# mkofinas/aether

Hardware: AMD Instinct MI355X
Metric: edge-messages/sec (forward, electrostatic N=20 batch=128 per GPU) (higher is better)
Workload: dtype f32; 1 GPU; electrostatic-2d-N20-B128; num_dims=2, nodes_per_graph=20, graphs_per_gpu=128, edges_per_gpu=48640, hidden=64, launch=hipgraph (10 steps per replay), parallelism=graphs sharded over 1 rank(s), no forward collective

## Files before the change

### aether_amd/_lib.py

```python
from __future__ import annotations

import ctypes as C
import os

HERE = os.path.dirname(os.path.abspath(__file__))
LIB_PATH = os.path.join(HERE, "libaether_hip.so")

PARAM_FIELDS = [
    ("field_w0", "field_net.net.0.weight"), ("field_b0", "field_net.net.0.bias"),
    ("field_w2", "field_net.net.2.weight"), ("field_b2", "field_net.net.2.bias"),
    ("field_w4", "field_net.net.4.weight"), ("field_b4", "field_net.net.4.bias"),
    ("field_emb", "field_net.class_embedding.weight"),
    ("l1_msg_w0", "gnn.layer_1.message_fn.0.weight"), ("l1_msg_b0", "gnn.layer_1.message_fn.0.bias"),
    ("l1_msg_w2", "gnn.layer_1.message_fn.2.weight"), ("l1_msg_b2", "gnn.layer_1.message_fn.2.bias"),
    ("l1_res_w", "gnn.layer_1.res.weight"), ("l1_res_b", "gnn.layer_1.res.bias"),
    ("l1_upd_w0", "gnn.layer_1.update_fn.0.weight"), ("l1_upd_b0", "gnn.layer_1.update_fn.0.bias"),
    ("l1_upd_w2", "gnn.layer_1.update_fn.2.weight"), ("l1_upd_b2", "gnn.layer_1.update_fn.2.bias"),
    ("ln_msg_w0", "gnn.layer_{}.message_fn.0.weight"), ("ln_msg_b0", "gnn.layer_{}.message_fn.0.bias"),
    ("ln_msg_w2", "gnn.layer_{}.message_fn.2.weight"), ("ln_msg_b2", "gnn.layer_{}.message_fn.2.bias"),
    ("ln_upd_w0", "gnn.layer_{}.update_fn.0.weight"), ("ln_upd_b0", "gnn.layer_{}.update_fn.0.bias"),
    ("ln_upd_w2", "gnn.layer_{}.update_fn.2.weight"), ("ln_upd_b2", "gnn.layer_{}.update_fn.2.bias"),
    ("out_w0", "gnn.out_mlp.0.weight"), ("out_b0", "gnn.out_mlp.0.bias"),
    ("out_w3", "gnn.out_mlp.3.weight"), ("out_b3", "gnn.out_mlp.3.bias"),
    ("out_w6", "gnn.out_mlp.6.weight"), ("out_b6", "gnn.out_mlp.6.bias"),
# ... 203 lines not shown
                                   [C.c_int, C.c_int, C.c_int, C.c_int] + [C.c_void_p] * 4 + [C.c_size_t, C.c_void_p]),
    "aether_sim_charged": (C.c_int, [C.c_void_p, C.c_void_p, C.c_void_p, C.c_void_p, C.c_int64, C.c_int, C.c_int, C.c_int,
                                     C.c_double, C.c_double, C.c_double, C.c_int, C.c_void_p, C.c_double, C.c_void_p,
                                     C.c_void_p, C.c_void_p]),
    "aether_rollout_dynamic_field": (C.c_int, [C.c_void_p, C.c_void_p, C.c_int, C.c_int64, C.c_int64, C.c_int] +
                                     [C.c_void_p] * 6 + [C.c_size_t, C.c_void_p, C.c_void_p, C.c_int, C.c_float, C.c_int,
                                                         C.c_void_p]),
    "aether_s2s_encoder_features": (C.c_int, [C.c_void_p, C.c_int, C.c_int, C.c_int, C.c_int, C.c_int64, C.c_int64] +
                                    [C.c_void_p] * 7 + [C.c_size_t, C.c_void_p, C.c_void_p]),
    "aether_s2s_lstm_step": (C.c_int, [C.c_void_p] * 4 + [C.c_int, C.c_int, C.c_int64] + [C.c_void_p] * 7),
    "aether_s2s_mlp_head": (C.c_int, [C.c_void_p, C.c_void_p, C.c_int, C.c_int, C.c_int, C.c_int, C.c_int64,
                                      C.c_void_p, C.c_void_p, C.c_void_p, C.c_void_p]),
    "aether_s2s_gumbel_hard": (C.c_int, [C.c_void_p, C.c_void_p, C.c_float, C.c_int, C.c_int64, C.c_void_p,
                                         C.c_void_p]),
    "aether_dynamic_field": (C.c_int, [C.c_void_p, C.c_int, C.c_int64, C.c_int, C.c_void_p, C.c_void_p, C.c_void_p,
                                       C.c_void_p, C.c_void_p]),
    "aether_forward_field": (C.c_int, [C.POINTER(AetherParams), C.c_int, C.c_int64, C.c_int64, C.c_void_p, C.c_void_p,
                                       C.c_void_p, C.c_void_p, C.c_void_p, C.c_void_p, C.POINTER(AetherGraphInfo),
                                       C.c_void_p, C.c_size_t, C.c_void_p, C.c_int, C.c_void_p]),
    "aether_debug_fetch": (C.c_int64, [C.c_char_p, C.c_int, C.c_int64, C.c_int64, C.c_void_p,
                                       C.c_void_p, C.c_void_p]),
    "aether_debug_split": (C.c_int, [C.c_void_p, C.c_int] + [C.c_void_p] * 5),
    "aether_debug_fused_packed_edge": (C.c_int, [C.c_int, C.c_int]),
    "aether_workspace_bytes_h": (C.c_size_t, [C.c_int64, C.c_int64, C.c_int, C.c_int, C.c_int]),
    "aether_dropout_mask_offset_h": (C.c_size_t, [C.c_int64, C.c_int64, C.c_int, C.c_int]),
    "aether_forward_h": (C.c_int, [C.POINTER(AetherParams), C.c_int, C.c_int, C.c_int64, C.c_int64, C.c_void_p, C.c_void_p,
                                   C.c_void_p, C.c_void_p, C.c_void_p, C.c_void_p, C.POINTER(AetherGraphInfo),
                                   C.c_void_p, C.c_size_t, C.c_void_p, C.c_int, C.c_void_p]),
    "aether_backward_h": (C.c_int, [C.POINTER(AetherParams), C.POINTER(AetherParams), C.c_int, C.c_int, C.c_int64,
                                    C.c_int64, C.c_void_p, C.c_void_p, C.c_void_p, C.c_void_p,
                                    C.POINTER(AetherGraphInfo), C.c_void_p, C.c_size_t, C.c_void_p, C.c_void_p,
                                    C.c_void_p]),
    "aether_backward_inputs_h": (C.c_int, [C.POINTER(AetherParams), C.c_int, C.c_int, C.c_int64, C.c_int64, C.c_void_p,
                                           C.c_void_p, C.c_void_p, C.c_void_p, C.POINTER(AetherGraphInfo), C.c_void_p,
                                           C.c_size_t, C.c_void_p, C.c_void_p, C.c_void_p, C.c_void_p, C.c_void_p,
                                           C.c_void_p, C.c_void_p]),
    "aether_rollout_h": (C.c_int, [C.POINTER(AetherParams), C.c_int, C.c_int, C.c_int64, C.c_int64, C.c_void_p, C.c_void_p,
                                   C.c_void_p, C.c_void_p, C.POINTER(AetherGraphInfo), C.c_void_p, C.c_size_t,
                                   C.c_void_p, C.c_int, C.c_float, C.c_int, C.c_void_p]),
    "aether_rollout_dynamic_field_h": (C.c_int, [C.c_void_p, C.c_void_p, C.c_int, C.c_int, C.c_int64, C.c_int64, C.c_int] +
                                       [C.c_void_p] * 6 + [C.c_size_t, C.c_void_p, C.c_void_p, C.c_int, C.c_float, C.c_int,
                                                           C.c_void_p]),
    "aether_debug_fetch_h": (C.c_int64, [C.c_char_p, C.c_int, C.c_int, C.c_int64, C.c_int64, C.c_void_p, C.c_void_p,
                                         C.c_void_p]),
    "aether_rollout_train_workspace_bytes": (C.c_size_t, [C.c_int64, C.c_int64, C.c_int, C.c_int, C.c_int]),
    "aether_rollout_train_forward": (C.c_int, [C.POINTER(AetherParams), C.c_int, C.c_int, C.c_int64, C.c_int64, C.c_void_p,
# ... 91 lines not shown
```

### aether_amd/csrc/aether_hip.hip

```cpp

#include <hip/hip_runtime.h>
#include <hipcub/hipcub.hpp>

#include <cstdint>
#include <cstdio>
#include <cstring>

#include "common.h"
#include "streamed.h"
#include "fused.h"
#include "backward.h"
#include "fused_bwd.h"
#include "edge_acc.h"
#include "input_grad.h"
#include "rollout_bwd.h"
#include "wide.h"
#include "seq2seq.h"
#include "s2s_filter.h"
#include "s2s_step.h"
#include "s2s_markov.h"
#include "s2s_charges.h"
#include "s2s_locs.h"
#include "s2s_dnri.h"
#include "dynfield.h"
// ... 1518 lines not shown
    if (name[0] == 'x' && name[1] >= '0' && name[1] <= '4' && !name[2])
        return copy2d((const float*)(ws + W.x[name[1] - '0']), n_nodes, H, 0, H);
    if (name[0] == 'e' && name[1] >= '1' && name[1] <= '4' && !name[2])
        return copy2d((const float*)(ws + W.e[name[1] - '1']), n_edges, H, 0, H);
    if (!strcmp(name, "efeat"))
        return copy2d((const float*)(ws + W.feat), n_edges, FPAD, 0, FPAD);
    return fail(AETHER_EINVAL, "debug_fetch: unknown name");
}

int aether_debug_split(const float* x, int n_tiles, uint16_t* hi, uint16_t* lo, int* on, float* scale, float* y) {
    if (!x || !hi || !lo || !on || !scale || !y) return fail(AETHER_EINVAL, "debug_split: null pointer");
    if (n_tiles < 0) return fail(AETHER_EINVAL, "debug_split: n_tiles");
    if (n_tiles == 0) return AETHER_OK;
    k_debug_split<<<dim3(1), dim3(64 * DEBUG_SPLIT_WAVES), 0, nullptr>>>(x, n_tiles, hi, lo, on, scale, y);
    HIP_OK(hipGetLastError());
    return AETHER_OK;
}

int aether_debug_fused_packed_edge(int wave, int lane) {
    if (wave < 0 || wave >= FUSED_PACK_WAVES || lane < 0 || lane >= FUSED_PACK_LANES) return -1;
    return fused_packed_edge(wave, lane);
}

#include "host_wide.inc"
#include "host_rollout_train.inc"

}
```

### aether_amd/csrc/common.h

```cpp
#pragma once
#include <hip/hip_runtime.h>
#include <cstdint>
#include <type_traits>
#include "../../include/aether_hip.h"

namespace {

typedef float f32x4 __attribute__((ext_vector_type(4)));
typedef float f32x2 __attribute__((ext_vector_type(2)));

constexpr int H = AETHER_HIDDEN;
constexpr int LDW = H + 8;
constexpr int FPAD = 32;
constexpr int LDF = FPAD + 8;
constexpr int LDST = H + 4;
constexpr float PI_F = 3.14159274101257324f;
constexpr float TWO_PI_F = 6.28318548202514648f;
constexpr float EPS_F = 1e-7f;

__device__ __forceinline__ void lds_barrier() { asm volatile("s_waitcnt lgkmcnt(0)\n\ts_barrier" ::: "memory"); }

__device__ __forceinline__ f32x4 mfma16(float a, float b, f32x4 c) {
    return __builtin_amdgcn_mfma_f32_16x16x4f32(a, b, c, 0, 0, 0);
}
// ... 502 lines not shown
    float c = cosf(theta), s = sinf(theta);
    if constexpr (D == 2) {
        R[0][0] = c; R[0][1] = -s; R[1][0] = s; R[1][1] = c;
    } else {
        float rho = sqrtf(v[0] * v[0] + v[1] * v[1] + v[2] * v[2]);
        float cz = v[2] / (rho + EPS_F);
        cz = fminf(fmaxf(cz, -1.0f), 1.0f);
        float phi = acosf(cz);
        float cp = cosf(phi), sp = sinf(phi);
        R[0][0] = cp * c; R[0][1] = -s;  R[0][2] = sp * c;
        R[1][0] = cp * s; R[1][1] = c;   R[1][2] = sp * s;
        R[2][0] = -sp;    R[2][1] = 0.f; R[2][2] = cp;
    }
#pragma unroll
    for (int a = 0; a < D; ++a) {
        float sv = 0.f, sf = 0.f;
#pragma unroll
        for (int b = 0; b < D; ++b) { sv += R[b][a] * v[b]; sf += R[b][a] * f[b]; }
        cv[a] = sv; cf[a] = sf;
    }
}

template <int D>
__device__ __forceinline__ void edge_features(const float* __restrict__ nj,
                                              const float* __restrict__ nir,
                                              const float* __restrict__ ea, float* __restrict__ o) {
    using NI = NodeInfo<D>;
    constexpr int O = D * (D - 1) / 2;
    float rel[D], rrel[D], rv[D], rf[D];
#pragma unroll
    for (int d = 0; d < D; ++d) rel[d] = nj[NI::P + d] - nir[NI::P + d];
#pragma unroll
    for (int a = 0; a < D; ++a) {
        float s0 = 0.f, s1 = 0.f, s2 = 0.f;
#pragma unroll
        for (int b = 0; b < D; ++b) {
            float rba = nir[NI::R + b * D + a];
            s0 += rba * rel[b];
            s1 += rba * nj[NI::V + b];
            s2 += rba * nj[NI::F + b];
        }
        rrel[a] = s0; rv[a] = s1; rf[a] = s2;
    }
    auto M = [&](int a, int c) {
        float s = 0.f;
#pragma unroll
// ... 42 lines not shown
```

### aether_amd/csrc/fused.h

```cpp
#pragma once
#include "common.h"
#include "fused_layout.h"
#include "fused_graph.h"
#include "fused_handoff.h"

namespace {

struct FusedDebug {
    float* nodeinfo; float* x[5]; float* e[4];
    float* n[4]; float* ps[3]; float* pr[3]; float* feat;
    int* flags;
    int* errword;
    const float* wimg;
    float* stamps;
    StepExtras step;
};
constexpr int FUSED_STAMPS = 512;

#ifdef AETHER_FUSED_STAMPS
#define FUSED_STAMP(id)                                                                          \
    do {                                                                                         \
        if (tid == 0 && blockIdx.x < 4096)                                                       \
            dbg.stamps[blockIdx.x * FUSED_STAMPS + (id)] = (float)(wall_clock64() - t_entry) * 0.01f; \
    } while (0)
#define FUSED_WSTAMP(layer_, r_, k_)                                                              \
    do {                                                                                         \
        if ((layer_) == 2 && lane == 0 && blockIdx.x < 4096 && wave < 16)                        \
            dbg.stamps[blockIdx.x * FUSED_STAMPS + 64 + wave * 24 + (r_) * 8 + (k_)] =            \
                (float)(__builtin_amdgcn_s_memtime() - c_entry);                                 \
    } while (0)
#define FUSED_WSTAMP_ROWS(layer_, r_)                                                             \
    do {                                                                                         \
        if ((layer_) == 2 && lane == 0 && blockIdx.x < 4096 && wave < 16)                        \
            dbg.stamps[blockIdx.x * FUSED_STAMPS + 352 + wave * 4 + (r_)] =                       \
                (float)(__builtin_amdgcn_s_memtime() - c_entry);                                 \
    } while (0)
#define FUSED_PSTAMP(k_, dep_)                                                                    \
    do {                                                                                         \
        asm volatile("v_mov_b32 %0, %0" : "+v"(dep_));                                           \
        if (wave == 0 && lane == 0 && blockIdx.x < 4096)                                         \
            dbg.stamps[blockIdx.x * FUSED_STAMPS + 400 + (k_)] =                                  \
                (float)(__builtin_amdgcn_s_memtime() - c_entry);                                 \
    } while (0)
#else
#define FUSED_STAMP(id)
#define FUSED_WSTAMP(layer_, r_, k_)
#define FUSED_WSTAMP_ROWS(layer_, r_)
#define FUSED_PSTAMP(k_, dep_)
#endif

template <int D, int NW, int ROUNDS, bool KEEP, bool GRAN = false>
__global__ void __launch_bounds__(NW * 64)
k_fused(AetherParams P, const float* __restrict__ x, const float* __restrict__ vel,
        const float* __restrict__ charges, const float* __restrict__ edge_attr_orig,
        const int32_t* __restrict__ perm, const int32_t* __restrict__ send_s,
        const int32_t* __restrict__ recv_s, const int32_t* __restrict__ rowptr,
        const FusedWG* __restrict__ wgdesc, const uint32_t* __restrict__ trec, const int4* __restrict__ ledge,
        const int32_t* __restrict__ nrange, FusedDebug dbg, float* __restrict__ out) {
    constexpr bool keep = KEEP;
    using NI = NodeInfo<D>;
    using L = FusedLds<NW, ROUNDS>;
    constexpr int THREADS = NW * 64;
    constexpr int FIN = 2 * D + 16;
    static_assert(NW == 8 || NW == 12, "waves 0-7 run the node phase; NW == 12 adds four waves that run step 3 (DESIGN.md 4.1)");
    static_assert(NW == 8 || (ROUNDS == 1 && !KEEP), "the 12-wave kernel owns one tile per wave and saves nothing for the backward");
    static_assert(!GRAN || NW == 12, "granules are the 12-wave kernel's hand-off");
    constexpr bool LATE = NW == 12 || ROUNDS == 2;
    constexpr bool EARLY = NW == 12;
    extern __shared__ __attribute__((aligned(16))) float smem[];
    float* wA = smem + L::WA;
    float* wB = smem + L::WB;
// ... 28 lines not shown
        const int total = nw_frag + FUSED_CBLK / 256;
        const int wv = __builtin_amdgcn_readfirstlane(wave);
        __builtin_assume(wv >= 0 && wv < NW);
        const int g_img = fused_wimg_offset(layer_, 0), g_cb = fused_cblk_offset(layer_);
        const int l_cb = L::CBLK + (layer_ & 1) * FUSED_CBLK;
        constexpr int MAXF = (32 + FUSED_CBLK / 256 + NW - 1) / NW;
#pragma unroll
        for (int j = 0; j < MAXF; ++j) {
            const int f = wv + NW * j;
            if (f < total) {
                const int img = f < na_frag ? f * 256 : FUSED_WIMG + (f - na_frag) * 256;
                const int soff = f < nw_frag ? g_img + img : g_cb + (f - nw_frag) * 256;
                const int doff = f < nw_frag ? L::WA + img : l_cb + (f - nw_frag) * 256;
                __builtin_amdgcn_global_load_lds(dbg.wimg + soff + lane * 4, (__attribute__((address_space(3))) void*)(smem + doff), 16, 0, 0);
            }
        }
    };
    dma_images(1);
    FUSED_STAMP(1);

    constexpr int FR = ROUNDS < 2 ? ROUNDS : 2;
    constexpr bool PACKED = NW == 12;
    constexpr bool FIMG = NW == 12;
    const int f_local = PACKED ? fused_packed_edge(wave, lane) : 16 * (NW * (lane >> 4) + wave) + (lane & 15);
    const bool f_have = (PACKED ? wave < FUSED_PACK_WAVES && lane < FUSED_PACK_LANES : lane < 16 * FR) && f_local < m;
    int4 f_e = make_int4(0, 0, 0, 0);
    f32x2 f_ea = {0.0f, 0.0f};
    int4 t_e[ROUNDS];
    unsigned seg_ends[ROUNDS];
    unsigned seg_rows[ROUNDS][4];
    {
        const int wv = __builtin_amdgcn_readfirstlane(wave);
#pragma unroll
        for (int r = 0; r < ROUNDS; ++r) {
            const int stile = NW * r + wv;
            const uint32_t* rec = trec + (size_t)(wg.tile0 + (stile < n_tiles ? stile : 0)) * FUSED_TREC;
            seg_ends[r] = stile < n_tiles ? __builtin_amdgcn_readfirstlane(rec[0]) : 0u;
#pragma unroll
            for (int w = 0; w < 4; ++w) seg_rows[r][w] = __builtin_amdgcn_readfirstlane(rec[2 + w]);
        }
    }
    const int aslot = (tid >> 4) & (FUSED_MAX_NODES - 1), ac4 = (tid & 15) * 4;
    int4 nr_rec;
    const int4* own_desc = reinterpret_cast<const int4*>(wgdesc + blockIdx.x);
    const int4* le_base = m > 0 ? ledge + eb : own_desc;
    const int4* nr_base = n > 0 ? reinterpret_cast<const int4*>(nrange) + nb : own_desc;
// ... 36 lines not shown
            int64_t g;
            float pz[D], vz[D], ef[D];
            float ch;
            float zc[6][3], a1[2][6];
            f32x4 w2f[2][2], w4f[2], acc1[2], acc2[2];
            f32x4 acc3 = f32x4{0.f, 0.f, 0.f, 0.f};
            float ar[4][2];
            f32x4 acc0[4];
            f32x4 fimg[FIMG ? FUSED_FIMG_CHUNKS : 1];
            if constexpr (FIMG) {
                const auto fimg_rsrc = __builtin_amdgcn_make_buffer_rsrc(const_cast<float*>(dbg.wimg) + fused_fimg_offset(), 0, FUSED_FIMG * 4, 0x00020000);
                p_ext = dbg.step.ext_field ? dbg.step.ext_field : x;
                asm volatile("" :: "s"(fimg_rsrc), "s"(p_ext), "s"(x), "s"(vel), "s"(charges), "s"(le_base), "s"(nr_base),
                             "s"(ea_base), "s"(qattr));
                node = 16 * wave + i;
                live = node < nv;
                g = vb + (live ? node : 0);
                FUSED_PSTAMP(0, f_e.x);
#pragma unroll
                for (int d = 0; d < D; ++d) { pz[d] = x[g * D + d]; vz[d] = vel[g * D + d]; ef[d] = p_ext[g * D + d]; }
                ch = charges[g];
#pragma unroll
                for (int c = 0; c < FUSED_FIMG_CHUNKS; ++c)
                    fimg[c] = __builtin_bit_cast(f32x4, __builtin_amdgcn_raw_buffer_load_b128(fimg_rsrc, lane * 16, c * 1024, 0));
            } else {
                const float* p_emb = P.field_emb; const float* p_w0 = P.field_w0; const float* p_b0 = P.field_b0;
                const float* p_w2 = P.field_w2; const float* p_b2 = P.field_b2; const float* p_w4 = P.field_w4;
                const float* p_b4 = P.field_b4; const float* p_rb = P.l1_res_b; const float* p_rw = P.l1_res_w;
                p_ext = dbg.step.ext_field ? dbg.step.ext_field : x;
                asm volatile("" :: "s"(p_emb), "s"(p_w0), "s"(p_b0), "s"(p_w2), "s"(p_b2), "s"(p_w4), "s"(p_b4), "s"(p_rb),
                             "s"(p_rw), "s"(p_ext), "s"(x), "s"(vel), "s"(charges), "s"(le_base), "s"(nr_base), "s"(ea_base),
                             "s"(qattr));
                node = 16 * wave + i;
                live = node < nv;
                g = vb + (live ? node : 0);
                FUSED_PSTAMP(0, f_e.x);
#pragma unroll
                for (int d = 0; d < D; ++d) { pz[d] = x[g * D + d]; vz[d] = vel[g * D + d]; ef[d] = p_ext[g * D + d]; }
                ch = charges[g];
#pragma unroll
                for (int s4 = 0; s4 < 6; ++s4) {
                    const int k = 4 * s4 + q;
                    const int ke = (k >= 2 * D && k < FIN) ? k - 2 * D : 0, kw = k < FIN ? k : 0;
#pragma unroll
                    for (int c = 0; c < 3; ++c)
                        zc[s4][c] = (4 * s4 + 3 >= 2 * D && 4 * s4 < FIN) ? p_emb[c * 16 + ke] : 0.0f;
#pragma unroll
// ... 13 lines not shown
#pragma unroll
                for (int mb = 0; mb < 4; ++mb) {
                    acc0[mb] = ld4(p_rb + 16 * mb + 4 * q);
#pragma unroll
                    for (int s4 = 0; s4 < 2; ++s4)
                        ar[mb][s4] = 4 * s4 < 2 * D ? p_rw[(16 * mb + i) * 3 * D + D + (4 * s4 + q < 2 * D ? 4 * s4 + q : 0)] : 0.0f;
                }
            }
            index_stage_a();
            __builtin_amdgcn_sched_barrier(0);
            __builtin_amdgcn_s_waitcnt(0x0F70);
            __builtin_amdgcn_sched_barrier(0);
            FUSED_PSTAMP(1, f_e.x);
            auto landed = [](auto v) { asm volatile("" :: "v"(v)); };
            auto landed4 = [](const int4& v) { asm volatile("" :: "v"(v.x), "v"(v.y), "v"(v.z), "v"(v.w)); };
            landed4(f_e); landed4(nr_rec);
#pragma unroll
            for (int r = 0; r < ROUNDS; ++r) landed4(t_e[r]);
#pragma unroll
            for (int d = 0; d < D; ++d) { landed(pz[d]); landed(vz[d]); landed(ef[d]); }
            landed(ch);
            if constexpr (FIMG) {
#pragma unroll
                for (int c = 0; c < FUSED_FIMG_CHUNKS; ++c) landed(fimg[c]);
                auto slot = [&](int s) { return fimg[s >> 2][s & 3]; };
#pragma unroll
                for (int mb = 0; mb < 2; ++mb) {
                    acc1[mb] = fimg[FI_ACC1 / 4 + mb]; acc2[mb] = fimg[FI_ACC2 / 4 + mb];
#pragma unroll
                    for (int a = 0; a < 2; ++a) w2f[mb][a] = fimg[FI_W2F / 4 + 2 * mb + a];
#pragma unroll
                    for (int s4 = 0; s4 < 6; ++s4) a1[mb][s4] = slot(FI_A1 + 6 * mb + s4);
                }
#pragma unroll
                for (int a = 0; a < 2; ++a) w4f[a] = fimg[FI_W4F / 4 + a];
                acc3 = fimg[FI_ACC3 / 4];
#pragma unroll
                for (int s4 = 0; s4 < 6; ++s4)
#pragma unroll
                    for (int c = 0; c < 3; ++c) zc[s4][c] = slot(FI_ZC + 3 * s4 + c);
#pragma unroll
                for (int mb = 0; mb < 4; ++mb) {
                    acc0[mb] = fimg[FI_ACC0 / 4 + mb];
#pragma unroll
                    for (int s4 = 0; s4 < 2; ++s4) ar[mb][s4] = slot(FI_AR + 2 * mb + s4);
                }
            } else {
#pragma unroll
                for (int s4 = 0; s4 < 6; ++s4) {
#pragma unroll
                    for (int c = 0; c < 3; ++c)
                        if (4 * s4 + 3 >= 2 * D && 4 * s4 < FIN) landed(zc[s4][c]);
#pragma unroll
                    for (int mb = 0; mb < 2; ++mb)
                        if (4 * s4 < FIN) landed(a1[mb][s4]);
                }
#pragma unroll
                for (int mb = 0; mb < 2; ++mb) { landed(acc1[mb]); landed(acc2[mb]); landed(w2f[mb][0]); landed(w2f[mb][1]); }
                landed(w4f[0]); landed(w4f[1]);
#pragma unroll
                for (int r = 0; r < D; ++r) landed(acc3[r]);
#pragma unroll
                for (int mb = 0; mb < 4; ++mb) {
                    landed(acc0[mb]);
#pragma unroll
                    for (int s4 = 0; s4 < 2; ++s4)
                        if (4 * s4 < 2 * D) landed(ar[mb][s4]);
                }
#pragma unroll
// ... 23 lines not shown
#pragma unroll
                for (int d = 0; d < D; ++d) { zk = k == d ? pz[d] : zk; zk = k == D + d ? vz[d] : zk; }
#pragma unroll
                for (int mb = 0; mb < 2; ++mb) acc1[mb] = mfma16(a1[mb][s4], zk, acc1[mb]);
            }
            f32x4 hh[2];
#pragma unroll
            for (int mb = 0; mb < 2; ++mb) hh[mb] = silu4(acc1[mb]);
            asm volatile("" : "+v"(f_e.y), "+v"(f_e.z), "+v"(f_e.w) : "v"(hh[0][0]));
            f_ea = index_stage_b();
#pragma unroll
            for (int a = 0; a < 2; ++a)
#pragma unroll
                for (int b = 0; b < 4; ++b)
#pragma unroll
                    for (int mb = 0; mb < 2; ++mb) acc2[mb] = mfma16(w2f[mb][a][b], hh[a][b], acc2[mb]);
#pragma unroll
            for (int mb = 0; mb < 2; ++mb) hh[mb] = silu4(acc2[mb]);
#pragma unroll
            for (int a = 0; a < 2; ++a)
#pragma unroll
                for (int b = 0; b < 4; ++b) acc3 = mfma16(w4f[a][b], hh[a][b], acc3);
            FUSED_PSTAMP(2, acc3[0]);
            if (q == 0 && live) {
                float f[D], R[D][D], cv[D], cf[D];
#pragma unroll
                for (int d = 0; d < D; ++d)
                    f[d] = dbg.step.ext_field ? ef[d] : acc3[d];
                node_frame<D>(vz, f, R, cv, cf);
                float* ni = ninfo + node * 24;
#pragma unroll
                for (int d = 0; d < D; ++d) {
                    ni[NI::P + d] = pz[d]; ni[NI::V + d] = vz[d]; ni[NI::F + d] = f[d];
                    ni[NI::CV + d] = cv[d]; ni[NI::CF + d] = cf[d];
#pragma unroll
                    for (int e = 0; e < D; ++e) ni[NI::R + d * D + e] = R[d][e];
                }
                if (keep && node >= off && node < off + n) {
                    float* gni = dbg.nodeinfo + (int64_t)(vb + node) * NI::STRIDE;
#pragma unroll
                    for (int t = 0; t < NI::STRIDE; ++t) gni[t] = t < NI::CF + D ? ni[t] : 0.0f;
                }
            }
            __builtin_amdgcn_wave_barrier();
            FUSED_PSTAMP(3, acc3[0]);
#pragma unroll
            for (int s4 = 0; s4 < 2; ++s4) {
                const int k = 4 * s4 + q;
                const float rk = (live && k < 2 * D) ? ninfo[node * 24 + NI::CV + k] : 0.0f;
#pragma unroll
                for (int mb = 0; mb < 4; ++mb) acc0[mb] = mfma16(ar[mb][s4], rk, acc0[mb]);
            }
            const int own = node - off;
            if (own >= 0 && own < n) {
#pragma unroll
                for (int mb = 0; mb < 4; ++mb) {
                    st4(xbuf + own * LDW + 16 * mb + 4 * q, acc0[mb]);
                    if (keep) st4(dbg.x[0] + (int64_t)(nb + own) * H + 16 * mb + 4 * q, acc0[mb]);
                }
            }
            FUSED_PSTAMP(4, acc0[3][0]);
        } else {
            index_stage_a();
            index_select();
            f_ea = index_stage_b();
            for (int idx = tid - 64 * vtiles; idx < (FUSED_MAX_NODES - n) * (H / 4); idx += THREADS - 64 * vtiles)
                st4(xbuf + (n + (idx >> 4)) * LDW + (idx & 15) * 4, f32x4{0.f, 0.f, 0.f, 0.f});
        }
        asm volatile("s_waitcnt vmcnt(0)" ::: "memory");
        lds_barrier();
    }
    FUSED_STAMP(2);

    int sl[ROUNDS], rl[ROUNDS];
    f32x4 e[ROUNDS][4];
    int ke[KEEP ? ROUNDS : 1];
    {
        float* scratch = smem + L::FEAT + wave * (L::FEAT_ROWS * LDF);
#pragma unroll
        for (int r0 = 0; r0 < ROUNDS; r0 += 2) {
            constexpr int PASS = 2;
            const int nr_pass = ROUNDS - r0 < PASS ? ROUNDS - r0 : PASS;
            if (PACKED ? wave < FUSED_PACK_WAVES && lane < FUSED_PACK_LANES : lane < 16 * nr_pass) {
                const int r = r0 + (lane >> 4), ii = lane & 15;
                const int local = PACKED ? f_local : 16 * (NW * r + wave) + ii;
                float o[FPAD];
                if (local < m) {
                    const int4 le = r0 == 0 ? f_e : ledge[eb + local];
                    const int k = le.x, ks = le.y, kr = le.z;
                    const float* nj = ninfo + (ks - vb) * 24;
                    const float* nr = ninfo + (kr - vb) * 24;
                    float njl[NI::STRIDE], nrl[NI::STRIDE];
#pragma unroll
                    for (int t = 0; t < NI::STRIDE; ++t) { njl[t] = nj[t]; nrl[t] = nr[t]; }
                    float eal[2];
                    if (dbg.step.qattr) {
                        float d2 = 0.0f;
#pragma unroll
                        for (int d = 0; d < D; ++d) {
                            const float df = njl[NI::P + d] - nrl[NI::P + d];
                            d2 += df * df;
                        }
                        eal[0] = r0 == 0 ? f_ea[0] * f_ea[1] : dbg.step.qattr[ks] * dbg.step.qattr[kr];
                        eal[1] = sqrtf(d2);
                    } else if (r0 == 0) {
                        eal[0] = f_ea[0]; eal[1] = f_ea[1];
                    } else {
                        const float* ea = edge_attr_orig + 2 * (int64_t)le.w;
                        eal[0] = ea[0]; eal[1] = ea[1];
                    }
                    edge_features<D>(njl, nrl, eal, o);
                } else {
#pragma unroll
                    for (int t = 0; t < FPAD; ++t) o[t] = 0.0f;
                }
#pragma unroll
                for (int t = 0; t < FPAD; t += 4)
// ... 601 lines not shown
```

### aether_amd/csrc/fused_layout.h

```cpp
#pragma once
#include "common.h"

namespace {

constexpr int FUSED_MAX_NODES = 32;
constexpr int FUSED_MAX_EDGES = 384;
constexpr int FUSED_MAX_TILES = FUSED_MAX_EDGES / 16;
constexpr int LDU = 2 * H + 8;
constexpr int FUSED_PACK_WAVES = 4, FUSED_PACK_LANES = 48;
__device__ __host__ constexpr int fused_packed_edge(int wave, int lane) { return FUSED_PACK_LANES * wave + lane; }
static_assert(FUSED_PACK_WAVES * FUSED_PACK_LANES == 12 * 16 && FUSED_PACK_LANES % 16 == 0, "every row of the twelve tiles has one builder");

constexpr int FUSED_WIMG = SPLIT_WIMG;
constexpr int FUSED_CBLK = 768;
constexpr int CB_B1 = 0;
constexpr int CB_B2 = 64;
constexpr int CB_B3 = 128;
constexpr int CB_B4 = 256;
constexpr int CB_B1N = 320;
constexpr int CB_OB3 = 384;
constexpr int CB_OB6 = 448;
constexpr int CB_OW6 = 512;
template <int NW, int ROUNDS> struct FusedLds {
    static constexpr int WSZ = FUSED_WIMG;
    static constexpr int WA = 0;
    static constexpr int WB = WA + WSZ;
    static constexpr int CBLK = WB + WSZ;
    static constexpr int XBUF = CBLK + 2 * FUSED_CBLK;
    static constexpr int NBUF = XBUF + FUSED_MAX_NODES * LDW;
    static constexpr int PS = NBUF + FUSED_MAX_NODES * LDW;
    static constexpr int PR = PS + FUSED_MAX_NODES * LDW;
    static constexpr int NINFO = PR + FUSED_MAX_NODES * LDW;
    static constexpr int PART_ROWS = ROUNDS == 3 ? FUSED_MAX_NODES + FUSED_MAX_TILES : 2 * FUSED_MAX_NODES + 16;
    static constexpr int PART = NINFO + FUSED_MAX_NODES * 24;
// ... 24 lines not shown
    static constexpr int XPC = UPC + 2 * SPLIT_PIECES;
    static constexpr int OPC = XPC + SPLIT_PIECES;
    static constexpr int PFLAG = OPC + SPLIT_PIECES;
    static_assert(NW != 12 || (NPC >= OBUF2 + FUSED_MAX_NODES * LDW && NPC >= UBUF + FUSED_MAX_NODES * LDU && PFLAG + 5 * 4 <= TOTAL && NPC % 4 == 0), "operand pieces");
    static_assert(FIELD_END <= TOTAL, "field scratch");
    static_assert(UBUF + FUSED_MAX_NODES * LDU <= TOTAL, "ubuf");
    static_assert(OBUF2 + FUSED_MAX_NODES * LDW <= TOTAL, "obuf");
    static_assert(TOTAL * 4 <= 160 * 1024, "LDS budget");
};

constexpr int FUSED_NIMG_W3 = 2 * 8 * 2 * 64 * 4, FUSED_NIMG_W4 = 2 * 4 * 4 * 64 * 4, FUSED_NIMG_WS = 2 * 4 * 2 * 64 * 4;
constexpr int FUSED_NIMG_LAYER = FUSED_NIMG_W3 + FUSED_NIMG_W4 + 2 * FUSED_NIMG_WS;
constexpr int FI_ACC1 = 0;
constexpr int FI_ACC2 = 8;
constexpr int FI_W2F = 16;
constexpr int FI_W4F = 32;
constexpr int FI_ACC3 = 40;
constexpr int FI_ACC0 = 44;
constexpr int FI_A1 = 60;
constexpr int FI_ZC = 72;
constexpr int FI_AR = 90;
constexpr int FI_END = 98;
constexpr int FUSED_FIMG_CHUNKS = (FI_END + 3) / 4;
constexpr int FUSED_FIMG = FUSED_FIMG_CHUNKS * 256;
constexpr int FUSED_WIMG_SPLIT = 8 * FUSED_WIMG + 4 * FUSED_NIMG_LAYER + 4 * FUSED_CBLK;
constexpr int FUSED_WIMG_SET = FUSED_WIMG_SPLIT + FUSED_FIMG;
constexpr int FUSED_SPLIT_BLOCKS = 8 + 4 * 6 + 1 + FUSED_FIMG_CHUNKS;
__device__ __host__ constexpr int fused_fimg_offset() { return FUSED_WIMG_SPLIT; }
__device__ __host__ constexpr int fused_wimg_offset(int layer, int which) { return ((layer - 1) * 2 + which) * FUSED_WIMG; }
__device__ __host__ constexpr int fused_nimg_offset(int layer, int which) {
    return 8 * FUSED_WIMG + (layer - 1) * FUSED_NIMG_LAYER +
           (which == 0 ? 0 : which == 1 ? FUSED_NIMG_W3 : which == 2 ? FUSED_NIMG_W3 + FUSED_NIMG_W4 : FUSED_NIMG_W3 + FUSED_NIMG_W4 + FUSED_NIMG_WS);
}
__device__ __host__ constexpr int fused_cblk_offset(int layer) { return 8 * FUSED_WIMG + 4 * FUSED_NIMG_LAYER + (layer - 1) * FUSED_CBLK; }

__device__ __forceinline__ float fused_cblk_value(const AetherParams& P, int nd, int layer, int c) {
    if (c < CB_B2) return layer == 1 ? P.l1_msg_b0[c] : 0.0f;
    if (c < CB_B3) return (layer == 1 ? P.l1_msg_b2 : P.ln_msg_b2[layer - 2])[c - CB_B2];
    if (c < CB_B4) return (layer == 1 ? P.l1_upd_b0 : P.ln_upd_b0[layer - 2])[c - CB_B3];
    if (c < CB_B1N) return (layer == 1 ? P.l1_upd_b2 : P.ln_upd_b2[layer - 2])[c - CB_B4];
    if (c < CB_OB3) return (layer < 4 ? P.ln_msg_b0[layer - 1] : P.out_b0)[c - CB_B1N];
    if (layer < 4) return 0.0f;
    if (c < CB_OB6) return P.out_b3[c - CB_OB3];
    if (c < CB_OB6 + 4) return c - CB_OB6 < nd ? P.out_b6[c - CB_OB6] : 0.0f;
    if (c >= CB_OW6 && c < CB_OW6 + nd * H) return P.out_w6[c - CB_OW6];
    return 0.0f;
// ... 95 lines not shown
```

### include/aether_hip.h

```cpp
#ifndef AETHER_HIP_H
#define AETHER_HIP_H

#include <stddef.h>
#include <stdint.h>

#ifdef __cplusplus
extern "C" {
#endif

#define AETHER_OK 0
#define AETHER_EINVAL (-1)
#define AETHER_EINDEX (-2)
#define AETHER_EHIP (-3)
#define AETHER_ESPACE (-4)

#define AETHER_HIDDEN 64

typedef struct AetherParams {
    float* field_w0; float* field_b0;
    float* field_w2; float* field_b2;
    float* field_w4; float* field_b4;
    float* field_emb;
    float* l1_msg_w0; float* l1_msg_b0;
    float* l1_msg_w2; float* l1_msg_b2;
// ... 44 lines not shown
                              int keep_for_backward);

int aether_forward(const AetherParams* params, int num_dims, int64_t n_nodes, int64_t n_edges,
                   const float* x, const float* vel, const float* charges,
                   const float* edge_attr_orig, const void* graph, const AetherGraphInfo* info,
                   void* workspace, size_t workspace_bytes, float* out, int flags, void* stream);

int aether_rollout(const AetherParams* params, int num_dims, int64_t n_nodes, int64_t n_edges,
                   const float* x0, const float* vel0, const float* charges, const void* graph,
                   const AetherGraphInfo* info, void* workspace, size_t workspace_bytes,
                   float* trajectory, int steps, float dt, int flags, void* stream);

int aether_backward(const AetherParams* params, const AetherParams* grads, int num_dims, int64_t n_nodes,
                    int64_t n_edges, const float* x, const float* vel, const float* charges,
                    const void* graph, const AetherGraphInfo* info, void* workspace, size_t workspace_bytes,
                    const float* grad_out, void* stream);

int64_t aether_debug_fetch(const char* name, int num_dims, int64_t n_nodes, int64_t n_edges,
                           const void* workspace, float* dst, void* stream);

int aether_debug_split(const float* x, int n_tiles, uint16_t* hi, uint16_t* lo, int* on, float* scale, float* y);

int aether_debug_fused_packed_edge(int wave, int lane);

typedef struct AetherDynFieldParams {
    const float* gate_w0; const float* gate_b0; const float* gate_w2; const float* gate_b2;
    const float* nn_w0; const float* nn_b0; const float* nn_w2; const float* nn_b2;
    const float* lin1_w; const float* lin1_b; const float* lin2_w; const float* lin2_b;
    const float* lin3_w; const float* lin3_b;
    const float* film1_w0; const float* film1_b0; const float* film1_w2; const float* film1_b2;
    const float* film1_w4; const float* film1_b4;
    const float* film2_w0; const float* film2_b0; const float* film2_w2; const float* film2_b2;
    const float* film2_w4; const float* film2_b4;
    const float* emb;
} AetherDynFieldParams;
int aether_dynamic_field(const AetherDynFieldParams* params, int num_dims, int64_t n_graphs, int nodes_per_graph,
                         const float* x, const float* vel, const float* charges, float* field, void* stream);
int aether_forward_field(const AetherParams* params, int num_dims, int64_t n_nodes, int64_t n_edges,
                         const float* x, const float* vel, const float* charges, const float* field,
                         const float* edge_attr_orig, const void* graph, const AetherGraphInfo* info,
                         void* workspace, size_t workspace_bytes, float* out, int flags, void* stream);
int aether_rollout_dynamic_field(const AetherParams* params, const AetherDynFieldParams* dyn_params, int num_dims,
                                 int64_t n_nodes, int64_t n_edges, int nodes_per_graph, const float* x0,
                                 const float* vel0, const float* charges, const void* graph,
                                 const AetherGraphInfo* info, void* workspace, size_t workspace_bytes,
                                 float* field_scratch, float* trajectory, int steps, float dt, int flags, void* stream);
// ... 601 lines not shown
```

Before: 6.519 billion edge-messages/s.

## Move node-frame and x0 embedding off field waves onto idle waves

In the 12-wave fused kernel, the field waves no longer compute the node rotation frames and the initial x0 embedding. Idle waves now compute the velocity frames while the index build runs, and four x0 waves each handle one 16-row block of the embedding MFMA after the barrier. The rotated force is recomputed per edge from R and F. This shortens the critical path of the field waves at the cost of redundant per-edge force rotation and extra loads on the other waves.

New measurement: 6.632 billion edge-messages/s (median of 6 runs). +1.7%, better.

```diff
diff --git a/aether_amd/_lib.py b/aether_amd/_lib.py
--- a/aether_amd/_lib.py
+++ b/aether_amd/_lib.py
@@ -249,6 +249,7 @@
                                        C.c_void_p, C.c_void_p]),
     "aether_debug_split": (C.c_int, [C.c_void_p, C.c_int] + [C.c_void_p] * 5),
     "aether_debug_fused_packed_edge": (C.c_int, [C.c_int, C.c_int]),
+    "aether_debug_fused_wave_role": (C.c_int, [C.c_int, C.c_int]),
     "aether_workspace_bytes_h": (C.c_size_t, [C.c_int64, C.c_int64, C.c_int, C.c_int, C.c_int]),
     "aether_dropout_mask_offset_h": (C.c_size_t, [C.c_int64, C.c_int64, C.c_int, C.c_int]),
     "aether_forward_h": (C.c_int, [C.POINTER(AetherParams), C.c_int, C.c_int, C.c_int64, C.c_int64, C.c_void_p, C.c_void_p,
diff --git a/aether_amd/csrc/aether_hip.hip b/aether_amd/csrc/aether_hip.hip
--- a/aether_amd/csrc/aether_hip.hip
+++ b/aether_amd/csrc/aether_hip.hip
@@ -1564,6 +1564,13 @@
     return fused_packed_edge(wave, lane);
 }
 
+int aether_debug_fused_wave_role(int what, int wave) {
+    if (wave < 0 || wave >= 12) return -1;
+    if (what == 0) return wave >= FUSED_FRAME_WAVE0 && fused_frame_tile(wave) < FUSED_MAX_NODES / 16 ? fused_frame_tile(wave) : -1;
+    if (what == 1) return wave >= FUSED_X0_WAVE0 && fused_x0_rowblock(wave) < FUSED_X0_WAVES ? fused_x0_rowblock(wave) : -1;
+    return -1;
+}
+
 #include "host_wide.inc"
 #include "host_rollout_train.inc"
 
diff --git a/aether_amd/csrc/common.h b/aether_amd/csrc/common.h
--- a/aether_amd/csrc/common.h
+++ b/aether_amd/csrc/common.h
@@ -548,6 +548,42 @@
 }
 
 template <int D>
+__device__ __forceinline__ void node_frame_vel(const float (&v)[D], float (&R)[D][D], float (&cv)[D]) {
+    float theta = atan2f(v[1], v[0]);
+    if (theta < 0.0f) theta += TWO_PI_F;
+    float c = cosf(theta), s = sinf(theta);
+    if constexpr (D == 2) {
+        R[0][0] = c; R[0][1] = -s; R[1][0] = s; R[1][1] = c;
+    } else {
+        float rho = sqrtf(v[0] * v[0] + v[1] * v[1] + v[2] * v[2]);
+        float cz = v[2] / (rho + EPS_F);
+        cz = fminf(fmaxf(cz, -1.0f), 1.0f);
+        float phi = acosf(cz);
+        float cp = cosf(phi), sp = sinf(phi);
+        R[0][0] = cp * c; R[0][1] = -s;  R[0][2] = sp * c;
+        R[1][0] = cp * s; R[1][1] = c;   R[1][2] = sp * s;
+        R[2][0] = -sp;    R[2][1] = 0.f; R[2][2] = cp;
+    }
+#pragma unroll
+    for (int a = 0; a < D; ++a) {
+        float sv = 0.f;
+#pragma unroll
+        for (int b = 0; b < D; ++b) sv += R[b][a] * v[b];
+        cv[a] = sv;
+    }
+}
+template <int D>
+__device__ __forceinline__ void node_frame_force(const float* __restrict__ R, const float* __restrict__ f, float* __restrict__ cf) {
+#pragma unroll
+    for (int a = 0; a < D; ++a) {
+        float sf = 0.f;
+#pragma unroll
+        for (int b = 0; b < D; ++b) sf += R[b * D + a] * f[b];
+        cf[a] = sf;
+    }
+}
+
+template <int D>
 __device__ __forceinline__ void edge_features(const float* __restrict__ nj,
                                               const float* __restrict__ nir,
                                               const float* __restrict__ ea, float* __restrict__ o) {
diff --git a/aether_amd/csrc/fused.h b/aether_amd/csrc/fused.h
--- a/aether_amd/csrc/fused.h
+++ b/aether_amd/csrc/fused.h
@@ -35,18 +35,20 @@
             dbg.stamps[blockIdx.x * FUSED_STAMPS + 352 + wave * 4 + (r_)] =                       \
                 (float)(__builtin_amdgcn_s_memtime() - c_entry);                                 \
     } while (0)
-#define FUSED_PSTAMP(k_, dep_)                                                                    \
+#define FUSED_PSTAMP_W(w_, k_, dep_)                                                              \
     do {                                                                                         \
         asm volatile("v_mov_b32 %0, %0" : "+v"(dep_));                                           \
-        if (wave == 0 && lane == 0 && blockIdx.x < 4096)                                         \
+        if (wave == (w_) && lane == 0 && blockIdx.x < 4096)                                      \
             dbg.stamps[blockIdx.x * FUSED_STAMPS + 400 + (k_)] =                                  \
                 (float)(__builtin_amdgcn_s_memtime() - c_entry);                                 \
     } while (0)
+#define FUSED_PSTAMP(k_, dep_) FUSED_PSTAMP_W(0, k_, dep_)
 #else
 #define FUSED_STAMP(id)
 #define FUSED_WSTAMP(layer_, r_, k_)
 #define FUSED_WSTAMP_ROWS(layer_, r_)
 #define FUSED_PSTAMP(k_, dep_)
+#define FUSED_PSTAMP_W(w_, k_, dep_)
 #endif
 
 template <int D, int NW, int ROUNDS, bool KEEP, bool GRAN = false>
@@ -121,6 +123,8 @@
     constexpr int FR = ROUNDS < 2 ? ROUNDS : 2;
     constexpr bool PACKED = NW == 12;
     constexpr bool FIMG = NW == 12;
+    constexpr bool FRAMES = NW == 12;
+    f32x4 x0_acc = f32x4{0.f, 0.f, 0.f, 0.f}, x0_ar = f32x4{0.f, 0.f, 0.f, 0.f};
     const int f_local = PACKED ? fused_packed_edge(wave, lane) : 16 * (NW * (lane >> 4) + wave) + (lane & 15);
     const bool f_have = (PACKED ? wave < FUSED_PACK_WAVES && lane < FUSED_PACK_LANES : lane < 16 * FR) && f_local < m;
     int4 f_e = make_int4(0, 0, 0, 0);
@@ -203,7 +207,8 @@
                 ch = charges[g];
 #pragma unroll
                 for (int c = 0; c < FUSED_FIMG_CHUNKS; ++c)
-                    fimg[c] = __builtin_bit_cast(f32x4, __builtin_amdgcn_raw_buffer_load_b128(fimg_rsrc, lane * 16, c * 1024, 0));
+                    if (fused_fimg_field_chunk(c))
+                        fimg[c] = __builtin_bit_cast(f32x4, __builtin_amdgcn_raw_buffer_load_b128(fimg_rsrc, lane * 16, c * 1024, 0));
             } else {
                 const float* p_emb = P.field_emb; const float* p_w0 = P.field_w0; const float* p_b0 = P.field_b0;
                 const float* p_w2 = P.field_w2; const float* p_b2 = P.field_b2; const float* p_w4 = P.field_w4;
@@ -263,7 +268,8 @@
             landed(ch);
             if constexpr (FIMG) {
 #pragma unroll
-                for (int c = 0; c < FUSED_FIMG_CHUNKS; ++c) landed(fimg[c]);
+                for (int c = 0; c < FUSED_FIMG_CHUNKS; ++c)
+                    if (fused_fimg_field_chunk(c)) landed(fimg[c]);
                 auto slot = [&](int s) { return fimg[s >> 2][s & 3]; };
 #pragma unroll
                 for (int mb = 0; mb < 2; ++mb) {
@@ -280,12 +286,7 @@
                 for (int s4 = 0; s4 < 6; ++s4)
 #pragma unroll
                     for (int c = 0; c < 3; ++c) zc[s4][c] = slot(FI_ZC + 3 * s4 + c);
-#pragma unroll
-                for (int mb = 0; mb < 4; ++mb) {
-                    acc0[mb] = fimg[FI_ACC0 / 4 + mb];
-#pragma unroll
-                    for (int s4 = 0; s4 < 2; ++s4) ar[mb][s4] = slot(FI_AR + 2 * mb + s4);
-                }
+                static_assert(FRAMES, "FI_ACC0 / FI_AR: the x0 waves' operands, loaded by them (P1's else branch)");
             } else {
 #pragma unroll
                 for (int s4 = 0; s4 < 6; ++s4) {
@@ -355,48 +356,87 @@
 #pragma unroll
                 for (int b = 0; b < 4; ++b) acc3 = mfma16(w4f[a][b], hh[a][b], acc3);
             FUSED_PSTAMP(2, acc3[0]);
-            if (q == 0 && live) {
-                float f[D], R[D][D], cv[D], cf[D];
-#pragma unroll
-                for (int d = 0; d < D; ++d)
-                    f[d] = dbg.step.ext_field ? ef[d] : acc3[d];
-                node_frame<D>(vz, f, R, cv, cf);
-                float* ni = ninfo + node * 24;
-#pragma unroll
-                for (int d = 0; d < D; ++d) {
-                    ni[NI::P + d] = pz[d]; ni[NI::V + d] = vz[d]; ni[NI::F + d] = f[d];
-                    ni[NI::CV + d] = cv[d]; ni[NI::CF + d] = cf[d];
-#pragma unroll
-                    for (int e = 0; e < D; ++e) ni[NI::R + d * D + e] = R[d][e];
-                }
-                if (keep && node >= off && node < off + n) {
-                    float* gni = dbg.nodeinfo + (int64_t)(vb + node) * NI::STRIDE;
-#pragma unroll
-                    for (int t = 0; t < NI::STRIDE; ++t) gni[t] = t < NI::CF + D ? ni[t] : 0.0f;
-                }
-            }
-            __builtin_amdgcn_wave_barrier();
-            FUSED_PSTAMP(3, acc3[0]);
-#pragma unroll
-            for (int s4 = 0; s4 < 2; ++s4) {
-                const int k = 4 * s4 + q;
-                const float rk = (live && k < 2 * D) ? ninfo[node * 24 + NI::CV + k] : 0.0f;
-#pragma unroll
-                for (int mb = 0; mb < 4; ++mb) acc0[mb] = mfma16(ar[mb][s4], rk, acc0[mb]);
-            }
-            const int own = node - off;
-            if (own >= 0 && own < n) {
-#pragma unroll
-                for (int mb = 0; mb < 4; ++mb) {
-                    st4(xbuf + own * LDW + 16 * mb + 4 * q, acc0[mb]);
-                    if (keep) st4(dbg.x[0] + (int64_t)(nb + own) * H + 16 * mb + 4 * q, acc0[mb]);
-                }
-            }
-            FUSED_PSTAMP(4, acc0[3][0]);
+            if constexpr (FRAMES) {
+                if (q == 0 && live) {
+#pragma unroll
+                    for (int d = 0; d < D; ++d)
+                        ninfo[node * 24 + NI::F + d] = dbg.step.ext_field ? ef[d] : acc3[d];
+                }
+                FUSED_PSTAMP(3, acc3[0]);
+            } else {
+                if (q == 0 && live) {
+                    float f[D], R[D][D], cv[D], cf[D];
+#pragma unroll
+                    for (int d = 0; d < D; ++d)
+                        f[d] = dbg.step.ext_field ? ef[d] : acc3[d];
+                    node_frame<D>(vz, f, R, cv, cf);
+                    float* ni = ninfo + node * 24;
+#pragma unroll
+                    for (int d = 0; d < D; ++d) {
+                        ni[NI::P + d] = pz[d]; ni[NI::V + d] = vz[d]; ni[NI::F + d] = f[d];
+                        ni[NI::CV + d] = cv[d]; ni[NI::CF + d] = cf[d];
+#pragma unroll
+                        for (int e = 0; e < D; ++e) ni[NI::R + d * D + e] = R[d][e];
+                    }
+                    if (keep && node >= off && node < off + n) {
+                        float* gni = dbg.nodeinfo + (int64_t)(vb + node) * NI::STRIDE;
+#pragma unroll
+                        for (int t = 0; t < NI::STRIDE; ++t) gni[t] = t < NI::CF + D ? ni[t] : 0.0f;
+                    }
+                }
+                __builtin_amdgcn_wave_barrier();
+                FUSED_PSTAMP(3, acc3[0]);
+#pragma unroll
+                for (int s4 = 0; s4 < 2; ++s4) {
+                    const int k = 4 * s4 + q;
+                    const float rk = (live && k < 2 * D) ? ninfo[node * 24 + NI::CV + k] : 0.0f;
+#pragma unroll
+                    for (int mb = 0; mb < 4; ++mb) acc0[mb] = mfma16(ar[mb][s4], rk, acc0[mb]);
+                }
+                const int own = node - off;
+                if (own >= 0 && own < n) {
+#pragma unroll
+                    for (int mb = 0; mb < 4; ++mb) {
+                        st4(xbuf + own * LDW + 16 * mb + 4 * q, acc0[mb]);
+                        if (keep) st4(dbg.x[0] + (int64_t)(nb + own) * H + 16 * mb + 4 * q, acc0[mb]);
+                    }
+                }
+                FUSED_PSTAMP(4, acc0[3][0]);
+            }
         } else {
+            const int ft = fused_frame_tile(wave), fnode = 16 * ft + i;
+            const bool fwave = FRAMES && ft >= 0 && ft < vtiles;
+            const bool flive = fwave && fnode < nv;
+            float pz[D], vz[D];
+            if constexpr (FRAMES) {
+                const auto fimg_rsrc = __builtin_amdgcn_make_buffer_rsrc(const_cast<float*>(dbg.wimg) + fused_fimg_offset(), 0, FUSED_FIMG * 4, 0x00020000);
+                const int64_t g = vb + (flive ? fnode : 0);
+#pragma unroll
+                for (int d = 0; d < D; ++d) { pz[d] = x[g * D + d]; vz[d] = vel[g * D + d]; }
+                const int mb = __builtin_amdgcn_readfirstlane(fused_x0_rowblock(wave)) & 3;
+                x0_acc = __builtin_bit_cast(f32x4, __builtin_amdgcn_raw_buffer_load_b128(fimg_rsrc, lane * 16, (FI_ACC0 / 4 + mb) * 1024, 0));
+                x0_ar = __builtin_bit_cast(f32x4, __builtin_amdgcn_raw_buffer_load_b128(fimg_rsrc, lane * 16, ((FI_AR + 2 * mb) >> 2) * 1024, 0));
+            }
             index_stage_a();
             index_select();
             f_ea = index_stage_b();
+            if constexpr (FRAMES) {
+#pragma unroll
+                for (int d = 0; d < D; ++d) asm volatile("" :: "v"(pz[d]), "v"(vz[d]));
+                FUSED_PSTAMP_W(FUSED_FRAME_WAVE0, 5, vz[0]);
+                if (flive && q == 0) {
+                    float R[D][D], cv[D];
+                    node_frame_vel<D>(vz, R, cv);
+                    float* ni = ninfo + fnode * 24;
+#pragma unroll
+                    for (int d = 0; d < D; ++d) {
+                        ni[NI::P + d] = pz[d]; ni[NI::V + d] = vz[d]; ni[NI::CV + d] = cv[d];
+#pragma unroll
+                        for (int e = 0; e < D; ++e) ni[NI::R + d * D + e] = R[d][e];
+                    }
+                }
+                FUSED_PSTAMP_W(FUSED_FRAME_WAVE0, 6, vz[0]);
+            }
             for (int idx = tid - 64 * vtiles; idx < (FUSED_MAX_NODES - n) * (H / 4); idx += THREADS - 64 * vtiles)
                 st4(xbuf + (n + (idx >> 4)) * LDW + (idx & 15) * 4, f32x4{0.f, 0.f, 0.f, 0.f});
         }
@@ -404,6 +444,46 @@
         lds_barrier();
     }
     FUSED_STAMP(2);
+
+    if constexpr (FRAMES) {
+        asm volatile("" :: "v"(x0_acc), "v"(x0_ar));
+        const int mb = __builtin_amdgcn_readfirstlane(fused_x0_rowblock(wave));
+        if (mb >= 0 && mb < FUSED_X0_WAVES) {
+            FUSED_PSTAMP_W(FUSED_X0_WAVE0, 7, x0_acc[0]);
+            const float ar[2] = {(mb & 1) ? x0_ar[0] : x0_ar[2], (mb & 1) ? x0_ar[1] : x0_ar[3]};
+            const int vtiles = (nv + 15) >> 4;
+            for (int t = 0; t < vtiles; ++t) {
+                const int lo = 16 * t > off ? 16 * t : off, hi = 16 * t + 16 < off + n ? 16 * t + 16 : off + n;
+                if (lo >= hi) continue;
+                const int node = 16 * t + i;
+                const bool live = node < nv;
+                const float* ni = ninfo + (live ? node : 0) * 24;
+                float rec[2 * D];
+#pragma unroll
+                for (int d = 0; d < D; ++d) rec[d] = ni[NI::CV + d];
+                {
+                    float Rl[D * D], fl[D];
+#pragma unroll
+                    for (int d = 0; d < D; ++d) fl[d] = ni[NI::F + d];
+#pragma unroll
+                    for (int d = 0; d < D * D; ++d) Rl[d] = ni[NI::R + d];
+                    node_frame_force<D>(Rl, fl, rec + D);
+                }
+                f32x4 acc = x0_acc;
+#pragma unroll
+                for (int s4 = 0; s4 < 2; ++s4) {
+                    const int k = 4 * s4 + q;
+                    float rk = 0.0f;
+#pragma unroll
+                    for (int kk = 4 * s4; kk < 4 * s4 + 4 && kk < 2 * D; ++kk) rk = (live && k == kk) ? rec[kk] : rk;
+                    acc = mfma16(ar[s4], rk, acc);
+                }
+                const int own = node - off;
+                if (own >= 0 && own < n) st4(xbuf + own * LDW + 16 * mb + 4 * q, acc);
+            }
+            FUSED_PSTAMP_W(FUSED_X0_WAVE0, 8, x0_acc[0]);
+        }
+    }
 
     int sl[ROUNDS], rl[ROUNDS];
     f32x4 e[ROUNDS][4];
@@ -426,6 +506,7 @@
                     float njl[NI::STRIDE], nrl[NI::STRIDE];
 #pragma unroll
                     for (int t = 0; t < NI::STRIDE; ++t) { njl[t] = nj[t]; nrl[t] = nr[t]; }
+                    if constexpr (FRAMES) node_frame_force<D>(nrl + NI::R, nrl + NI::F, nrl + NI::CF);
                     float eal[2];
                     if (dbg.step.qattr) {
                         float d2 = 0.0f;
diff --git a/aether_amd/csrc/fused_layout.h b/aether_amd/csrc/fused_layout.h
--- a/aether_amd/csrc/fused_layout.h
+++ b/aether_amd/csrc/fused_layout.h
@@ -10,6 +10,11 @@
 constexpr int FUSED_PACK_WAVES = 4, FUSED_PACK_LANES = 48;
 __device__ __host__ constexpr int fused_packed_edge(int wave, int lane) { return FUSED_PACK_LANES * wave + lane; }
 static_assert(FUSED_PACK_WAVES * FUSED_PACK_LANES == 12 * 16 && FUSED_PACK_LANES % 16 == 0, "every row of the twelve tiles has one builder");
+constexpr int FUSED_FRAME_WAVE0 = 2, FUSED_X0_WAVE0 = 4, FUSED_X0_WAVES = 4;
+__device__ __host__ constexpr int fused_frame_tile(int wave) { return wave - FUSED_FRAME_WAVE0; }
+__device__ __host__ constexpr int fused_x0_rowblock(int wave) { return wave - FUSED_X0_WAVE0; }
+static_assert(FUSED_FRAME_WAVE0 >= FUSED_MAX_NODES / 16 && FUSED_FRAME_WAVE0 + FUSED_MAX_NODES / 16 <= 12 && FUSED_X0_WAVE0 + FUSED_X0_WAVES <= 12 &&
+              FUSED_X0_WAVES * 16 == H, "frame waves behind the field waves, one x0 wave per 16 of the H rows");
 
 constexpr int FUSED_WIMG = SPLIT_WIMG;
 constexpr int FUSED_CBLK = 768;
@@ -80,6 +85,13 @@
 constexpr int FI_AR = 90;
 constexpr int FI_END = 98;
 constexpr int FUSED_FIMG_CHUNKS = (FI_END + 3) / 4;
+static_assert(FI_ACC0 % 4 == 0 && FI_AR % 4 == 2, "an x0 wave's operands: one whole chunk and half of another");
+__device__ __host__ constexpr bool fused_fimg_x0_slot(int s) { return (s >= FI_ACC0 && s < FI_A1) || (s >= FI_AR && s < FI_END); }
+__device__ __host__ constexpr bool fused_fimg_field_chunk(int c) {
+    for (int r = 0; r < 4; ++r)
+        if (4 * c + r < FI_END && !fused_fimg_x0_slot(4 * c + r)) return true;
+    return false;
+}
 constexpr int FUSED_FIMG = FUSED_FIMG_CHUNKS * 256;
 constexpr int FUSED_WIMG_SPLIT = 8 * FUSED_WIMG + 4 * FUSED_NIMG_LAYER + 4 * FUSED_CBLK;
 constexpr int FUSED_WIMG_SET = FUSED_WIMG_SPLIT + FUSED_FIMG;
diff --git a/include/aether_hip.h b/include/aether_hip.h
--- a/include/aether_hip.h
+++ b/include/aether_hip.h
@@ -90,6 +90,8 @@
 int aether_debug_split(const float* x, int n_tiles, uint16_t* hi, uint16_t* lo, int* on, float* scale, float* y);
 
 int aether_debug_fused_packed_edge(int wave, int lane);
+
+int aether_debug_fused_wave_role(int what, int wave);
 
 typedef struct AetherDynFieldParams {
     const float* gate_w0; const float* gate_b0; const float* gate_w2; const float* gate_b2;
```
